# skmhrk1209/GANSynth

Measured on AMD Instinct MI355X. Metric: G+D step images/sec at 128x1024x2 mel+IF, higher is better.
Workload: dtype bf16; 1 GPU; BASELINE.json configs[1]: fully grown PGGAN 128x1024x2 G+D iteration (D update + G update, R1 + mode-seeking), per-GPU batch 8, random-init weights; global_batch=8, parallelism=dp1, launch=hipGraph replay, forked branches, forked_branches=True

## Files before the change

gansynth_amd/_lib.py:

```python
import ctypes
import os
from ctypes import c_char_p, c_double, c_float, c_int, c_int64, c_size_t, c_void_p, POINTER

_HERE = os.path.dirname(os.path.abspath(__file__))
LIB_PATH = os.path.join(_HERE, "libgansynth_hip.so")

GS_F32, GS_BF16 = 0, 1
ACT_NONE, ACT_LRELU, ACT_TANH = 0, 1, 2
ACT_LRELU_BITS, ACT_WRITE_BITS = 5, 16
PREP_CONV_FWD, PREP_CONV_BWD_DATA, PREP_CONVT_FWD, PREP_CONVT_BWD_DATA = 0, 1, 2, 3
CONV_FWD, CONV_BWD_DATA, CONV_BWD_WEIGHT = 0, 1, 2

P, I, F, L, Z = c_void_p, c_int, c_float, c_int64, c_size_t

SIGNATURES = {
    "gs_last_error": (c_char_p, []),
    "gs_version": (I, []),
    "gs_init": (I, []),
    "gs_streams_create": (I, [I, POINTER(P)]),
    "gs_streams_destroy": (I, [I, POINTER(P)]),
    "gs_prof_enable": (I, [I]),
    "gs_prof_collect": (I, [POINTER(c_int), POINTER(c_double), POINTER(c_double)]),
    "gs_prof_roofline": (I, [ctypes.c_double, ctypes.c_double, P, P, P]),
    "gs_prof_records": (I, [I, P, P, P, P, P]),
    "gs_comm_available": (I, []),
    "gs_comm_unique_id": (I, [P]),
    "gs_comm_init": (I, [POINTER(P), I, I, P]),
    "gs_comm_destroy": (I, [P]),
    "gs_comm_count": (I, [P, POINTER(I)]),
    "gs_allreduce_sum_f32": (I, [P, P, ctypes.c_int64, P]),
    "gs_comm_set_marker_us": (I, [P, ctypes.c_double]),
    "gs_broadcast_f32": (I, [P, P, ctypes.c_int64, I, P]),
    "gs_conv2d_workspace_bytes": (Z, [I, I, I, I, I, I, I, I, I]),
    "gs_conv2d_fwd": (I, [P, P, P, I, I, I, I, I, I, I, F, I, I, P, Z, P]),
    "gs_conv2d_fwd_bias_act": (I, [P, P, P, P, I, I, I, I, I, I, I, F, I, I, I, P, Z, P]),
    "gs_conv2d_bwd_data": (I, [P, P, P, I, I, I, I, I, I, I, F, I, I, P, Z, P]),
    "gs_conv2d_fwd_bias_act_norm": (I, [P, P, P, P, P, I, I, I, I, I, I, I, F, I, F, I, I, P, Z, P]),
    "gs_conv2d_transpose_s2_fwd_bias_act_norm": (I, [P, P, P, P, P, I, I, I, I, I, F, I, F, I, I, P, Z, P]),
    "gs_conv2d_fwd_mask": (I, [P, P, P, I, P, I, I, I, I, I, I, I, F, I, I, P, Z, P]),
    "gs_conv2d_bwd_data_mask": (I, [P, P, P, I, P, I, I, I, I, I, I, I, F, I, I, P, Z, P]),
    "gs_conv2d_bwd_weight": (I, [P, P, P, I, I, I, I, I, I, I, F, I, I, P, Z, P]),
    "gs_conv2d_bwd_weight_bias": (I, [P, P, P, P, I, I, I, I, I, I, I, F, I, I, P, Z, P]),
    "gs_conv2d_bwd_weight_bias_partial": (I, [P, P, P, P, I, I, I, I, I, I, I, F, I, I, P, Z, P, P]),
    "gs_conv2d_transpose_s2_bwd_weight_partial": (I, [P, P, P, I, I, I, I, I, F, I, I, P, Z, P, P]),
    "gs_wgrad_reduce_batch": (I, [P, I, P]),
    "gs_conv2d_bwd_weight_bias_multi": (I, [P, P, P, I, ctypes.c_uint, P, P, I, I, I, I, I, I, I, F, I, I, P, Z, P, P]),
    "gs_conv2d_transpose_s2_bwd_weight_multi": (I, [P, P, P, I, P, I, I, I, I, I, F, I, I, P, Z, P, P]),
    "gs_conv_wgrad_jobs_workspace_bytes": (Z, [P, I]),
    "gs_conv_wgrad_jobs": (I, [P, I, P, Z, P]),
    "gs_wgrad_cu_cap": (I, [I]),
    "gs_conv2d_transpose_s2_workspace_bytes": (Z, [I, I, I, I, I, I, I]),
    "gs_conv2d_transpose_s2_fwd": (I, [P, P, P, I, I, I, I, I, F, I, I, P, Z, P]),
    "gs_conv2d_transpose_s2_fwd_bias_act": (I, [P, P, P, P, I, I, I, I, I, F, I, I, I, P, Z, P]),
    "gs_conv2d_transpose_s2_bwd_data": (I, [P, P, P, I, I, I, I, I, F, I, I, P, Z, P]),
    "gs_conv2d_bwd_data_pnbwd_is_fused": (I, [I, I, I, I, I, I, I, I, I]),
    "gs_conv2d_fwd_pnbwdbwd_is_fused": (I, [I, I, I, I, I, I, I, I, I]),
    "gs_units_bias_act_to_nhwc": (I, [P, P, P, P, I, I, I, I, I, P]),
    "gs_nhwc_act_bwd_to_units": (I, [P, P, P, I, I, I, I, I, P]),
    "gs_conv2d_fwd_pnbwdbwd": (I, [P, P, P, P, I, F, P, P, I, I, I, I, I, I, I, F, I, I, P, Z, P]),
    "gs_conv2d_transpose_s2_fwd_pnbwdbwd": (I, [P, P, P, P, I, F, P, P, I, I, I, I, I, F, I, I, P, Z, P]),
    "gs_conv2d_bwd_data_pnbwd": (I, [P, P, P, P, I, F, P, I, I, I, I, I, I, I, F, I, I, P, Z, P]),
    "gs_conv2d_transpose_s2_bwd_data_pnbwd": (I, [P, P, P, P, I, F, P, I, I, I, I, I, F, I, I, P, Z, P]),
    "gs_conv2d_transpose_s2_bwd_weight": (I, [P, P, P, I, I, I, I, I, F, I, I, P, Z, P]),
    "gs_dense_fwd_workspace_bytes": (Z, [I, I, I]),
    "gs_dense_fwd": (I, [P, P, P, I, I, I, F, I, P, Z, P]),
    "gs_dense_fwd_bias_act": (I, [P, P, P, P, I, I, I, F, I, I, P, Z, P]),
    "gs_dense_fwd_bias_act_nhwc": (I, [P, P, P, P, I, I, I, I, F, I, I, P, Z, P]),
    "gs_dense_bwd_data": (I, [P, P, P, I, I, I, F, I, P]),
    "gs_dense_bwd_weight": (I, [P, P, P, I, I, I, F, I, I, P]),
    "gs_dense_fwd_nhwc": (I, [P, P, P, I, I, I, I, F, I, P, Z, P]),
    "gs_dense_bwd_data_nhwc": (I, [P, P, P, I, I, I, I, F, I, P]),
    "gs_dense_bwd_weight_nhwc": (I, [P, P, P, I, I, I, I, F, I, I, P]),
    "gs_embedding_fwd": (I, [P, P, P, I, I, I, F, I, P]),
    "gs_embedding_onehot_fwd": (I, [P, P, P, P, I, I, I, F, I, P]),
    "gs_embedding_bwd": (I, [P, P, P, I, I, I, F, I, P]),
    "gs_bias_act_fwd": (I, [P, P, P, L, I, I, I, P]),
    "gs_act_bwd": (I, [P, P, P, L, I, I, P]),
    "gs_act_bwd_bias": (I, [P, P, P, P, L, I, I, I, I, P, Z, P]),
    "gs_tanh_bwd_bwd": (I, [P, P, P, P, L, I, P]),
    "gs_channel_sum_workspace_bytes": (Z, [L, I]),
    "gs_channel_sum": (I, [P, P, L, I, I, I, P, Z, P]),
    "gs_bias_partial_rows": (I, [I, L, I, I]),
    "gs_channel_fold_batch_workspace_bytes": (Z, [P, I]),
# ... 99 lines not shown
```

gansynth_amd/config.py:

```python
import os

KNOBS = {
    "GS_TORCH_COLLECTIVES": ("operational", "gradient all-reduce through torch.distributed's communicator instead of the library's own (gs_comm_*)"),
    "GS_NO_GRAPH_ALLREDUCE": ("operational", "no RCCL collective inside captured graphs: eager all-reduce behind each replay (bench.DP_LADDER's tamer modes)"),
    "GS_FORK_PROBE": ("operational", "auto | always | never: probe a forked hipGraph replay in a child process before the first forked capture "
                                     "(auto: only on HIP builds the workaround was not debugged on, fork_probe._forked_replay_ok)"),
    "GS_FORK_PROBED": ("operational", "(set by the probe for child processes: ok | died)"),
    "GS_FORK_PROBE_TIMEOUT_S": ("operational", "budget of that probe, seconds (600)"),
    "GS_LEVEL_STREAMS": ("operational", "throw-away streams alive while a graph is instantiated (128; capture.Capture._leveled_queues)"),
    "GS_COMM_MARKER_US": ("operational", "tests / profiles at world size 1: the one-rank all-reduce becomes a kernel that holds its stream this long "
                                         "(read once per communicator, comm.RcclComm; gs_comm_set_marker_us)"),
    "GS_CAPTURE_MODE": ("operational", "debugging: force torch.cuda.graph's capture_error_mode"),
    "GS_DEBUG_POISON_WS": ("operational", "debugging: kernel workspaces start as NaN bit patterns"),
    "GS_CHECK_FUSION": ("operational", "debugging: every fused cross-node form also runs its unfused definition and the two are compared"),
    "GS_FORK_EAGER": ("operational", "tests: the forked branches with eager launches on two streams"),
    "GS_NO_FORK_MARKS": ("operational", "debugging: branches start where they are opened, not at their marks"),
    "GS_NO_FORK": ("schedule", "no parallel branches in the runs' graphs (5.9 against 5.2 ms; also taken when GPU_MAX_HW_QUEUES != 4 or the probe fails)"),
    "GS_NO_MERGED_RUNS": ("schedule", "part A of the generator run NOT inside the discriminator run's graph (5.13 against 4.99 ms)"),
    "GS_NO_FUSED_ITERATION": ("schedule", "two graphs per iteration with eager optimizer steps between them (neutral on one GPU; data parallel both "
                                          "all-reduces are then the last node of a graph)"),
    "GS_OVERLAP_REDUCE": ("schedule", "data parallel: round 4's four-graph iteration, each all-reduce on a forked branch beside part A of the other run "
                                      "(hides both collectives; +0.7 ms at world size 1)"),
    "GS_NO_OVERLAP_REDUCE": ("schedule", "(overrides GS_OVERLAP_REDUCE)"),
    "GS_DEBUG_DP_BUCKET": ("operational", "print the range the first message of a two-step discriminator all-reduce covers"),
    "GS_DP_BUCKET_D": ("schedule", "data parallel: the discriminator's gradient all-reduced in two steps, ~98 % of it beside the end of its backward (300-us stand-ins: -0.09 ... -0.14 ms fully grown, +0.15 in a fade-in)"),
    "GS_EARLY_FLUSH_DIV": ("schedule", "a layer is 'large' from 1/DIV of the full resolution's pixels (16)"),
    "GS_EARLY_FLUSH_CUS": ("schedule", "CUs the early weight-gradient contraction is sized for (192; 160 / 224 / 256 within noise, round 6)"),
    "GS_D_TAIL_LEVELS": ("schedule", "levels of the discriminator's tail run over [real; fake] as one batch when the runs do not fork (3)"),
    "GS_NO_EARLY_FLUSH": ("ablation", "weight gradients of the full-chip levels contracted at the end of the run only"),
    "GS_NO_DEFERRED_REDUCE": ("ablation", "every weight gradient contracted where autograd produces it"),
    "GS_NO_DEFERRED_FOLDS": ("ablation", "bias-gradient partial rows folded by their producers"),
    "GS_NO_WGRAD_GROUPS": ("ablation", "no grouped weight-gradient launches"),
    "GS_NO_SPLIT_G_LOSS": ("ablation", "the generator's loss as one launch over both halves: the mode-seeking second-order pass waits for the discriminator's forward"),
    "GS_NO_SPLIT_FINAL_FLUSH": ("ablation", "the final weight-gradient contraction of a run on one stream (HBM-bound and MFMA-bound jobs one after the other)"),
    "GS_NO_FUSED_LOSSES": ("ablation", "per-sample loss algebra in torch instead of the one-launch loss heads"),
    "GS_NO_D_TAIL_BATCH": ("ablation", "real and fake pass through the discriminator's tail separately (no-fork schedule)"),
    "GS_NO_FUSED_NORM": ("ablation", "pixel norm as its own node behind every generator conv"),
    "GS_NO_NORM_EPILOGUE": ("ablation", "no pixel norm in conv epilogues"),
    "GS_NO_NORM_BWD_EPILOGUE": ("ablation", "no previous-block norm backward in data-gradient epilogues"),
    "GS_NO_NORM_BWD2_EPILOGUE": ("ablation", "no second-order norm kernel in the forward-on-cotangent conv"),
    "GS_NO_NORM_BWD_BIAS": ("ablation", "bias sums outside the norm's backward"),
    "GS_NO_MASK_BITS": ("ablation", "leaky-relu masks read as the bf16 activations themselves, not as the sign bits stored behind them"),
    "GS_NO_PREMASK": ("ablation", "activation derivative never folded into the consuming data-gradient kernel"),
    "GS_NO_PREMASK_GRAPH": ("ablation", "... not across autograd nodes"),
    "GS_NO_PREMASK_GRAPH2": ("ablation", "... not in second-order graphs"),
    "GS_NO_PARAMS_ONLY": ("ablation", "leaf activations receive gradients like tf.gradients would not ask for"),
    "GS_NO_DERIVED_SLICES": ("ablation", "the 257-channel conv's weight slices copied on every use"),
# ... 19 lines not shown
```

gansynth_amd/csrc/conv_igemm.hip:

```cpp
#include <type_traits>
#include "conv_shared.h"
#include "gs_prof.h"

#ifndef GS_WGRAD_THIN_PREFETCH
#define GS_WGRAD_THIN_PREFETCH 1
#endif

extern "C" int gs_pixel_norm_fwd(const void* x, void* y, int64_t p, int c, float eps, int dtype, void* stream);
extern "C" int gs_pack_act_bits(void* z, int64_t p, int c, int dtype, void* stream);
extern "C" int gs_pixel_norm_bwd_fused(const void* g, const void* x, const void* addend, void* gx, int64_t p, int c, float eps, int pre_act, int post_act, int dtype,
                                       void* stream);
extern "C" int gs_pixel_norm_bwd_bwd_fused(const void* gg, const void* g, const void* x, void* out, void* out_g, int64_t p, int c, float eps, int pre_act,
                                           int dtype, void* stream);

namespace gs {

typedef float f32x16 __attribute__((ext_vector_type(16)));
typedef float f32x4 __attribute__((ext_vector_type(4)));
typedef __bf16 bf16x8 __attribute__((ext_vector_type(8)));


template <typename T> struct Mma;
template <> struct Mma<float> {
    typedef f32x4 frag_t;
// ... 1419 lines not shown
    if (slice < ntiles) {
        tile_setup(slice);
#pragma unroll
        for (int q = 0; q < NPIECE; ++q) issue_piece(q, 0);
    }
    constexpr int PPG = (NPIECE + NG - 1) / NG;
    for (int tile = slice; tile < ntiles; tile += nslices) {
        const bool more = tile + nslices < ntiles;
        wait_vmcnt(0);
        block_barrier();
        do_bias = bias_next;
        if (more) tile_setup(tile + nslices);
        const unsigned char* const xpl = lds_raw + buf * BUF + it * XPL;
        const unsigned char* const gpl = lds_raw + buf * BUF + 2 * XPL + ot * GPL;
        load_group(0, 0, xpl, gpl);
        __builtin_amdgcn_sched_barrier(0);
        static_for<NG>([&](auto gc) __attribute__((always_inline)) { GS_WG_GROUP_STEP(decltype(gc)::value, more, xpl, gpl, buf ^ 1); });
        block_barrier();
        buf ^= 1;
    }
    const long pstride = 9L * IC * OC + (with_bias ? OC : 0);
    if (bias_wave) {
        const float tot = swap32_sum(accb);
        if (hi == 0) part[(long)slice * pstride + 9L * IC * OC + oc0 + ot * 32 + l31] = tot;
    }
#pragma unroll
    for (int t = 0; t < 9; ++t) {
        float* dst = part + (long)slice * pstride + ((long)t * IC + ic0 + it * 32) * OC + oc0 + ot * 32 + l31;
#pragma unroll
        for (int r = 0; r < 16; ++r) dst[(long)((r & 3) + 8 * (r >> 2) + 4 * hi) * OC] = acc[t][r];
    }
}

#ifndef GS_SK_ROW128
#define GS_SK_ROW128 1
#endif
#ifndef GS_SK_FRONT_S1
#define GS_SK_FRONT_S1 0
#endif
#ifndef GS_SK_FRONT_S2
#define GS_SK_FRONT_S2 1
#endif
template <int MODE, int TW, bool SPEC>
__global__ __launch_bounds__(SPEC ? 512 : 256) void conv_wgrad_bf16_2x2_sk_kernel(const SkGroup g, float* __restrict__ part) {
    constexpr bool S2 = MODE == MODE_S2;
    constexpr int NP = S2 ? 64 : 256;
    constexpr int TH = NP / TW;
    constexpr int PH = patch_dim<MODE>(TH), PW = patch_dim<MODE>(TW);
    constexpr int S = S2 ? 2 : 1;
    constexpr bool R128 = GS_SK_ROW128 != 0;
    constexpr int XRG = R128 ? (PH * PW + 7) / 8 : (PH * PW + 15) / 16;
    constexpr int GRG = R128 ? NP / 8 : NP / 16;
    constexpr int XK = (XRG + 3) / 4, GK = GRG / 4;
    constexpr int XPL = R128 ? 0 : XK * 4096, GPL = R128 ? 0 : NP * 64;
    constexpr int XT = R128 ? XK * 4096 : 2 * XK * 4096, GT = NP * 128;
    constexpr int BUF = XT + GT;
    constexpr int NPIECE = R128 ? XK + GK : 2 * XK + 2 * GK;
    constexpr int XROWB = R128 ? 128 : 64, GROWB = XROWB;
    extern __shared__ __attribute__((aligned(16))) unsigned char lds_raw[];
    const unsigned a_base = (unsigned)(uintptr_t)lds_raw;

    const int tid = threadIdx.x;
    const int lane = tid & 63, hi = lane >> 5, l31 = lane & 31;
    const int wv8 = __builtin_amdgcn_readfirstlane(tid >> 6);
    const bool loader = SPEC && wv8 >= 4, issuer = !SPEC || loader, computer = !SPEC || !loader;
    const int wv = wv8 & 3;
    const int it = wv >> 1, ot = wv & 1;
    const int t_row = (lane & 15) >> 2;
    const int t_col = (((lane >> 4) & 1) * 16 + (lane & 3) * 4) * 2;
    const long nb = gridDim.x, total = g.total_units;
    const int U0 = (int)((blockIdx.x * total) / nb), U1 = (int)(((blockIdx.x + 1) * total) / nb);
    if (U0 >= U1) return;

    constexpr int RPP = R128 ? 8 : 16;
    const int p_row = R128 ? lane >> 3 : lane >> 2;
    int x_ly[XK], x_lx[XK], x_voff[XK], x_sw[XK];
#pragma unroll
// ... 167 lines not shown
                if (more) {
#pragma unroll
                    for (int q = 0; q < NPIECE; ++q) issue_piece(q, buf ^ 1);
                }
            } else {
                load_group(0, 0, xpl, gpl);
                __builtin_amdgcn_sched_barrier(0);
                static_for<NG>([&](auto gc) __attribute__((always_inline)) { GS_WG_GROUP_STEP(decltype(gc)::value, false, xpl, gpl, buf ^ 1); });
            }
        } else {
            load_group(0, 0, xpl, gpl);
            __builtin_amdgcn_sched_barrier(0);
            static_for<NG>([&](auto gc) __attribute__((always_inline)) { GS_WG_GROUP_STEP(decltype(gc)::value, more, xpl, gpl, buf ^ 1); });
        }
        block_barrier();
        buf ^= 1;
        if (leave && computer) {
            float* const dst0 = part + (long)(blockIdx.x + run_c) * GS_SK_PSTRIDE;
            if (bias_wave_c) {
                const float tot = swap32_sum(accb);
                if (hi == 0) dst0[9 * 4096 + ot * 32 + l31] = tot;
            }
            accb = 0.f;
#pragma unroll
            for (int t = 0; t < 9; ++t) {
                float* dst = dst0 + (t * 64 + it * 32) * 64 + ot * 32 + l31;
#pragma unroll
                for (int r = 0; r < 16; ++r) {
                    dst[((r & 3) + 8 * (r >> 2) + 4 * hi) * 64] = acc[t][r];
                    acc[t][r] = 0.f;
                }
            }
        }
    }
}

__global__ __launch_bounds__(256) void wgrad_sk_reduce_kernel(const SkGroup g, const float* __restrict__ part) {
    constexpr int L = 4, EPB = 64;
    __shared__ float4 red[256];
    const int r = blockIdx.y;
    int j = 0;
    while (j + 1 < g.njobs && r >= g.job[j + 1].run_base) ++j;
    const SkJob& q = g.job[j];
    const int ct = r - q.run_base;
    const int ic0 = (ct % q.n_ict) * 64, oc0 = (ct / q.n_ict) * 64;
    const long s0 = (long)q.unit_base + (long)ct * q.ntiles;
    const int b0 = sk_block_of(s0, g.nblocks, g.total_units), b1 = sk_block_of(s0 + q.ntiles - 1, g.nblocks, g.total_units);
    const int e = blockIdx.x * EPB + (threadIdx.x % EPB);
    const int sl = threadIdx.x / EPB;
    const bool live = e < GS_SK_PSTRIDE / 4;
    const bool is_bias = e >= 9 * 1024;
    if (blockIdx.x * EPB >= 9 * 1024 && !(q.gb && ic0 == 0)) return;
    const float* const base = part + (long)r * GS_SK_PSTRIDE + (long)e * 4;
    float4 a0 = make_float4(0.f, 0.f, 0.f, 0.f), a1 = a0, a2 = a0, a3 = a0;
    if (live) {
        int b = b0 + sl;
        for (; b + 3 * L <= b1; b += 4 * L) {
            const float4 v0 = *reinterpret_cast<const float4*>(base + (long)b * GS_SK_PSTRIDE);
            const float4 v1 = *reinterpret_cast<const float4*>(base + (long)(b + L) * GS_SK_PSTRIDE);
            const float4 v2 = *reinterpret_cast<const float4*>(base + (long)(b + 2 * L) * GS_SK_PSTRIDE);
            const float4 v3 = *reinterpret_cast<const float4*>(base + (long)(b + 3 * L) * GS_SK_PSTRIDE);
            a0.x += v0.x; a0.y += v0.y; a0.z += v0.z; a0.w += v0.w;
            a1.x += v1.x; a1.y += v1.y; a1.z += v1.z; a1.w += v1.w;
            a2.x += v2.x; a2.y += v2.y; a2.z += v2.z; a2.w += v2.w;
            a3.x += v3.x; a3.y += v3.y; a3.z += v3.z; a3.w += v3.w;
        }
        for (; b <= b1; b += L) {
            const float4 v0 = *reinterpret_cast<const float4*>(base + (long)b * GS_SK_PSTRIDE);
            a0.x += v0.x; a0.y += v0.y; a0.z += v0.z; a0.w += v0.w;
        }
    }
    a0.x += a2.x; a0.y += a2.y; a0.z += a2.z; a0.w += a2.w;
    a1.x += a3.x; a1.y += a3.y; a1.z += a3.z; a1.w += a3.w;
    red[threadIdx.x] = make_float4(a0.x + a1.x, a0.y + a1.y, a0.z + a1.z, a0.w + a1.w);
    __syncthreads();
    if (sl != 0 || !live) return;
    float4 s = make_float4(0.f, 0.f, 0.f, 0.f);
#pragma unroll
    for (int k = 0; k < L; ++k) {
        const float4 v = red[threadIdx.x + k * EPB];
        s.x += v.x; s.y += v.y; s.z += v.z; s.w += v.w;
    }
    if (is_bias) {
        if (!(q.gb && ic0 == 0)) return;
        float4* o = reinterpret_cast<float4*>(q.gb + oc0 + (e - 9 * 1024) * 4);
        const float4 old = q.accumulate ? *o : make_float4(0.f, 0.f, 0.f, 0.f);
        *o = make_float4(old.x + s.x, old.y + s.y, old.z + s.z, old.w + s.w);
        return;
    }
    const int t = e >> 10, i = (e >> 4) & 63, j4 = (e & 15) * 4;
    const float al = q.alpha;
    if (!q.transpose) {
        float4* o = reinterpret_cast<float4*>(q.gw + ((long)t * q.ICld + ic0 + i) * q.OC + oc0 + j4);
        const float4 old = q.accumulate ? *o : make_float4(0.f, 0.f, 0.f, 0.f);
        *o = make_float4(old.x + s.x * al, old.y + s.y * al, old.z + s.z * al, old.w + s.w * al);
    } else {
        const float v[4] = {s.x, s.y, s.z, s.w};
#pragma unroll
        for (int c = 0; c < 4; ++c) {
            float* o = q.gw + ((long)t * q.OC + oc0 + j4 + c) * q.IC + ic0 + i;
            *o = q.accumulate ? *o + v[c] * al : v[c] * al;
        }
    }
}


static int g_num_cus = 0;
static int num_cus() {
    if (g_num_cus == 0) {
        int dev = 0, n = 0;
        if (hipGetDevice(&dev) == hipSuccess && hipDeviceGetAttribute(&n, hipDeviceAttributeMultiprocessorCount, dev) == hipSuccess && n > 0)
            g_num_cus = n;
        else
            g_num_cus = 256;
    }
    return g_num_cus;
}
static int g_wgrad_cu_cap = 0;
static int wgrad_cus() {
    const int n = num_cus();
    return g_wgrad_cu_cap > 0 && g_wgrad_cu_cap < n ? g_wgrad_cu_cap : n;
}

#ifndef GS_MAX_BLOCKS_PER_CU
#define GS_MAX_BLOCKS_PER_CU 2
#endif
#ifndef GS_SMALL_D
#define GS_SMALL_D 2
#endif
template <typename T, int MODE, int A, int B, int TW, int TG, bool RESIDENT = false, int D = 2, int NORM = 0, int RB = 64, bool SPEC = false, bool BITS = false>
static int launch_igemm(ConvP p, hipStream_t st) {
    if constexpr (!BITS && sizeof(T) == 2 && NORM == 0) {
        if (p.mask_bits || p.bits_out) return launch_igemm<T, MODE, A, B, TW, TG, RESIDENT, D, NORM, RB, SPEC, true>(p, st);
    }
    constexpr int NP = 128 * B;
    constexpr int TH = NP / TW;
// ... 445 lines not shown
int wgrad_sk_tile_width(int Wb) {
    static const bool tw16 = getenv("GS_SK_TW16") != nullptr;
    return (Wb >= 32 || !tw16) ? 32 : 16;
}
void wgrad_sk_job_geometry(int mode, int tw, int N, SkJob& q) {
    const int np = mode == MODE_S2 ? 64 : 256;
    const int th = np / tw;
    q.tiles_x = cdiv(q.Wb, tw);
    q.tiles_y = cdiv(q.Hb, th);
    q.ntiles = N * q.tiles_x * q.tiles_y;
    q.n_ict = q.IC / 64;
    q.nct = q.n_ict * (q.OC / 64);
}
void wgrad_sk_plan(int mode, SkGroup& g) {
    long units = 0;
    int runs = 0;
    for (int j = 0; j < g.njobs; ++j) {
        g.job[j].unit_base = (int)units;
        g.job[j].run_base = runs;
        units += (long)g.job[j].nct * g.job[j].ntiles;
        runs += g.job[j].nct;
    }
    g.total_units = (int)units;
    g.total_runs = runs;
    static const int upb_env = getenv("GS_SK_UNITS_PER_BLOCK") ? atoi(getenv("GS_SK_UNITS_PER_BLOCK")) : 0;
    static const int upb2_env = getenv("GS_SK_UNITS_PER_BLOCK_S2") ? atoi(getenv("GS_SK_UNITS_PER_BLOCK_S2")) : 0;
    const int upb = mode == MODE_S2 ? (upb2_env > 0 ? upb2_env : 4) : (upb_env > 0 ? upb_env : 2);
    long nb = units / upb;
    if (nb > wgrad_cus()) nb = wgrad_cus();
    if (nb < 1) nb = 1;
    g.nblocks = (int)nb;
}
size_t wgrad_sk_bytes(const SkGroup& g) { return align256((size_t)(g.nblocks + g.total_runs) * GS_SK_PSTRIDE * sizeof(float)); }

int run_wgrad_sk(int mode, int tw, const SkGroup& g, void* ws, size_t ws_bytes, hipStream_t st) {
    if (g.njobs < 1 || g.njobs > GS_SK_MAX_JOBS) return fail(GS_ERR_ARG, "conv wgrad group: %d jobs", g.njobs);
    if (ws_bytes < wgrad_sk_bytes(g)) return fail(GS_ERR_WORKSPACE, "conv wgrad group: workspace %zu < %zu", ws_bytes, wgrad_sk_bytes(g));
    if ((long)g.total_units <= 0) return 0;
    float* part = reinterpret_cast<float*>(ws);
    double flops = 0.0, bytes = 0.0;
    int images = 0;
    for (int j = 0; j < g.njobs; ++j) {
        const SkJob& q = g.job[j];
        const int N = q.srcs.n_end[GS_WGRAD_MAX_SRC - 1];
        images += N;
        flops += 2.0 * 9.0 * (double)N * q.Hb * q.Wb * q.IC * q.OC;
        bytes += ((double)N * q.Hi * q.Wi * q.IC + (double)N * q.Hb * q.Wb * q.OC) * 2.0 + 9.0 * q.IC * q.OC * 4.0;
    }
    {
        ProfScope ps(st, flops, bytes, 20 + mode, g.njobs, tw, g.nblocks, g.total_units, g.total_runs, images, 1);
#define GS_WGSK(M, TWV, SP)                                                                                              \
    do {                                                                                                                \
        constexpr int np_ = (M == MODE_S2 ? 64 : 256), th_ = np_ / TWV;                                                 \
        constexpr int lds_ = 2 * (2 * ((((patch_dim<M>(th_) * patch_dim<M>(TWV) + 15) / 16 + 3) / 4) * 4096 + np_ * 64));  \
        auto kern_ = conv_wgrad_bf16_2x2_sk_kernel<M, TWV, SP>;                                                         \
        static bool set_ = false;                                                                                       \
        if (!set_) {                                                                                                    \
            if (hipFuncSetAttribute(reinterpret_cast<const void*>(kern_), hipFuncAttributeMaxDynamicSharedMemorySize, lds_) != hipSuccess) \
                return fail(GS_ERR_HIP, "conv wgrad group: cannot reserve %d bytes of dynamic LDS", lds_);              \
            set_ = true;                                                                                                \
        }                                                                                                               \
        hipLaunchKernelGGL(kern_, dim3((unsigned)g.nblocks), dim3(SP ? 512 : 256), lds_, st, g, part);                  \
    } while (0)
        static const int spec_env = getenv("GS_SK_SPEC") ? atoi(getenv("GS_SK_SPEC")) : 0;
        const bool spec = spec_env == 1 || (spec_env == 2 && mode == MODE_S1);
        if (spec) {
            if (mode == MODE_S1) { if (tw == 32) GS_WGSK(MODE_S1, 32, true); else GS_WGSK(MODE_S1, 16, true); }
            else { if (tw == 32) GS_WGSK(MODE_S2, 32, true); else GS_WGSK(MODE_S2, 16, true); }
        } else {
            if (mode == MODE_S1) { if (tw == 32) GS_WGSK(MODE_S1, 32, false); else GS_WGSK(MODE_S1, 16, false); }
            else { if (tw == 32) GS_WGSK(MODE_S2, 32, false); else GS_WGSK(MODE_S2, 16, false); }
        }
#undef GS_WGSK
    }
    GS_CHECK_LAUNCH();
    hipLaunchKernelGGL(wgrad_sk_reduce_kernel, dim3((GS_SK_PSTRIDE / 4 + 63) / 64, (unsigned)g.total_runs), dim3(256), 0, st, g, part);
    GS_CHECK_LAUNCH();
    return 0;
}

}

extern "C" int gs_wgrad_cu_cap(int cap) {
    const int was = gs::g_wgrad_cu_cap;
    gs::g_wgrad_cu_cap = cap < 0 ? 0 : cap;
    return was;
}
extern "C" int gs_prof_enable(int on) {
    gs::g_prof.on = on != 0;
    gs::g_prof.burst = on > 1 ? on : 1;
    gs::g_prof.used = 0;
    gs::g_prof.flops = 0.0;
    return 0;
}

extern "C" int gs_prof_roofline(double peak_tflops, double peak_gbps, double* total_bytes, double* roof_ms, double* roof_ms_hbm_bound) {
    double bytes = 0.0, roof = 0.0, roof_hbm = 0.0;
    for (int i = 0; i < gs::g_prof.used; ++i) {
        if (gs::g_prof.ldesc[i][0] >= 10) continue;
        const double tf = gs::g_prof.lflops[i] / (peak_tflops * 1e12) * 1e3, tb = gs::g_prof.lbytes[i] / (peak_gbps * 1e9) * 1e3;
        bytes += gs::g_prof.lbytes[i];
        roof += tf > tb ? tf : tb;
        if (tb >= tf) roof_hbm += tb;
    }
    if (total_bytes) *total_bytes = bytes;
    if (roof_ms) *roof_ms = roof;
    if (roof_ms_hbm_bound) *roof_ms_hbm_bound = roof_hbm;
    return 0;
}

extern "C" int gs_prof_records(int max_records, int* n, double* ms, double* flops, double* bytes, int* desc) {
    int k = 0;
    for (int i = 0; i < gs::g_prof.used && k < max_records; ++i, ++k) {
// ... 29 lines not shown
```

gansynth_amd/kernels.py:

```python
import contextlib
import ctypes
import os

import numpy as np
import torch

from . import config
from . import _lib
from ._lib import GS_BF16, GS_F32

CL = torch.channels_last


def _dt(t):
    if t.dtype == torch.float32:
        return GS_F32
    if t.dtype == torch.bfloat16:
        return GS_BF16
    raise TypeError(f"unsupported activation dtype {t.dtype}")


def _act(x):
    if x.dim() == 4:
        return x if x.is_contiguous(memory_format=CL) else x.contiguous(memory_format=CL)
# ... 30 lines not shown
            and t.untyped_storage().nbytes() == t.numel() * 2 + t.numel() // 8)


def _mask_act(mask, mask_act):
    return _lib.ACT_LRELU_BITS if (mask_act == _lib.ACT_LRELU and _has_bits(mask)) else int(mask_act)


def _stream():
    return ctypes.c_void_p(torch.cuda.current_stream().cuda_stream)


_POISON = config.flag("GS_DEBUG_POISON_WS")


def _ws(nbytes, device):
    if _POISON:
        return torch.full((max(int(nbytes), 256),), 0xFF, dtype=torch.uint8, device=device)
    return torch.empty(max(int(nbytes), 256), dtype=torch.uint8, device=device)


def _rows_cols(x):
    if x.dim() == 4:
        n, c, h, w = x.shape
        return n * h * w, c
    return x.shape[0], x.shape[1]


class HipKernels(object):
    def __init__(self):
        self.lib = _lib.load()
        if not torch.cuda.is_available():
            raise _lib.GansynthHipError("gansynth_amd needs a HIP device (torch.cuda.is_available() is False)")
        _lib.check(self.lib.gs_init(), "gs_init")
        self._param_ranges = []
        self._wcache = {}
        self._prep_tables = {}
        self._derived = {}
        self._folds = None
        self._pending = None
        self._guarding = False
        self._last_writer = {}
        self._early = None
        self._seen = None
        self._expected = {}
        self._tag = None
        self._complete = None

    def register_param_buffer(self, flat):
        self._param_ranges.append([flat.data_ptr(), flat.numel() * flat.element_size(), 0])

    def invalidate_weights(self, flat=None):
        ptr = None if flat is None else flat.data_ptr()
        for rng in self._param_ranges:
            if ptr is None or rng[0] <= ptr < rng[0] + rng[1]:
                rng[2] += 1

    def _weight_ws(self, w, tag, nbytes, plan=None):
        ptr = w.data_ptr()
        rng = next((r for r in self._param_ranges if r[0] <= ptr < r[0] + r[1]), None)
        if rng is None:
            return _ws(nbytes, w.device), 0
        key, stamp = (ptr, tag), (rng[2], w._version)
        ent = self._wcache.get(key)
        if ent is not None and ent[0].numel() >= nbytes:
            if ent[1] == stamp:
                return ent[0], 1
# ... 1095 lines not shown
```

include/gansynth_hip.h:

```cpp
#ifndef GANSYNTH_HIP_H
#define GANSYNTH_HIP_H

#include <stddef.h>
#include <stdint.h>

#ifdef __cplusplus
extern "C" {
#endif

enum { GS_F32 = 0, GS_BF16 = 1 };
enum { GS_OK = 0, GS_ERR_ARG = -1, GS_ERR_HIP = -2, GS_ERR_UNSUPPORTED = -3, GS_ERR_WORKSPACE = -4 };
enum { GS_ACT_NONE = 0, GS_ACT_LRELU = 1, GS_ACT_TANH = 2 };
enum { GS_ACT_LRELU_BITS = 5, GS_ACT_WRITE_BITS = 16 };
enum { GS_CONV_FWD = 0, GS_CONV_BWD_DATA = 1, GS_CONV_BWD_WEIGHT = 2 };

const char* gs_last_error(void);
int gs_version(void);
int gs_init(void);
int gs_streams_create(int n, void** streams);
int gs_streams_destroy(int n, void** streams);

int gs_prof_enable(int on);
int gs_prof_collect(int* launches, double* total_ms, double* total_flops);
int gs_prof_roofline(double peak_tflops, double peak_gbps, double* total_bytes, double* roof_ms, double* roof_ms_hbm_bound);
// ... 65 lines not shown
    int32_t ic_ld;
} GsWgradReduce;
int gs_conv2d_bwd_weight_bias_partial(const void* x, const void* gy, float* gw_hwio, float* gb, int n, int h, int w, int ci, int co,
                                      int ksize, int stride, float alpha, int accumulate, int dtype, void* ws, size_t ws_bytes,
                                      GsWgradReduce* pending, void* stream);
int gs_conv2d_transpose_s2_bwd_weight_partial(const void* x, const void* gy, float* gw_hwio, int n, int h, int w, int ci, int co,
                                              float alpha, int accumulate, int dtype, void* ws, size_t ws_bytes,
                                              GsWgradReduce* pending, void* stream);
int gs_wgrad_reduce_batch(const GsWgradReduce* pending, int n, void* stream);
#define GS_WGRAD_MAX_SOURCES 4
int gs_conv2d_bwd_weight_bias_multi(const void* const* xs, const void* const* gys, const int* ns, int nsrc, unsigned bias_mask, float* gw_hwio,
                                    float* gb, int n, int h, int w, int ci, int co, int ksize, int stride, float alpha, int accumulate,
                                    int dtype, void* ws, size_t ws_bytes, GsWgradReduce* pending, void* stream);
int gs_conv2d_transpose_s2_bwd_weight_multi(const void* const* xs, const void* const* gys, const int* ns, int nsrc, float* gw_hwio, int n, int h,
                                            int w, int ci, int co, float alpha, int accumulate, int dtype, void* ws, size_t ws_bytes,
                                            GsWgradReduce* pending, void* stream);

typedef struct GsWgradJob {
    const void* x[GS_WGRAD_MAX_SOURCES];
    const void* gy[GS_WGRAD_MAX_SOURCES];
    int32_t n[GS_WGRAD_MAX_SOURCES];
    int32_t nsrc;
    uint32_t bias_mask;
    float* gw;
    float* gb;
    int32_t h, w, ci, co, ksize, stride, transposed;
    float alpha;
    int32_t accumulate, dtype;
    int32_t gw_ci_stride;
} GsWgradJob;
size_t gs_conv_wgrad_jobs_workspace_bytes(const GsWgradJob* jobs, int njobs);
int gs_conv_wgrad_jobs(const GsWgradJob* jobs, int njobs, void* ws, size_t ws_bytes, void* stream);
int gs_wgrad_cu_cap(int cap);

enum { GS_PREP_CONV_FWD = 0, GS_PREP_CONV_BWD_DATA = 1, GS_PREP_CONVT_FWD = 2, GS_PREP_CONVT_BWD_DATA = 3 };
typedef struct GsPrepDesc {
    const float* w_hwio;
    void* ws;
    int32_t map, ci, co, ksize, stride, dtype;
} GsPrepDesc;
int gs_weight_prep_batch(const GsPrepDesc* descs, int n, void* stream);

size_t gs_dense_fwd_workspace_bytes(int b, int in, int out);
int gs_dense_fwd(const void* x, const float* w, void* y, int b, int in, int out, float alpha, int dtype,
                 void* ws, size_t ws_bytes, void* stream);
int gs_dense_bwd_data(const void* gy, const float* w, void* gx, int b, int in, int out, float alpha, int dtype, void* stream);
int gs_dense_bwd_weight(const void* x, const void* gy, float* gw, int b, int in, int out, float alpha, int accumulate, int dtype,
                        void* stream);
int gs_dense_fwd_bias_act(const void* x, const float* w, const float* bias, void* y, int b, int in, int out, float alpha, int act,
                          int dtype, void* ws, size_t ws_bytes, void* stream);
int gs_dense_fwd_nhwc(const void* x, const float* w, void* y, int b, int c, int hw, int out, float alpha, int dtype,
                      void* ws, size_t ws_bytes, void* stream);
int gs_dense_fwd_bias_act_nhwc(const void* x, const float* w, const float* bias, void* y, int b, int c, int hw, int out, float alpha,
                               int act, int dtype, void* ws, size_t ws_bytes, void* stream);
int gs_dense_bwd_data_nhwc(const void* gy, const float* w, void* gx, int b, int c, int hw, int out, float alpha, int dtype, void* stream);
int gs_dense_bwd_weight_nhwc(const void* x, const void* gy, float* gw, int b, int c, int hw, int out, float alpha, int accumulate,
                             int dtype, void* stream);

int gs_embedding_fwd(const int64_t* idx, const float* w, void* y, int b, int rows, int units, float alpha, int dtype, void* stream);
int gs_embedding_onehot_fwd(const void* labels, const float* w, void* y, int64_t* idx_out, int b, int rows, int units, float alpha, int dtype, void* stream);
int gs_embedding_bwd(const int64_t* idx, const void* gy, float* gw, int b, int rows, int units, float alpha, int dtype, void* stream);

int gs_bias_act_fwd(const void* x, const float* bias, void* y, int64_t p, int c, int act, int dtype, void* stream);
int gs_act_bwd(const void* g, const void* y, void* gx, int64_t numel, int act, int dtype, void* stream);
int gs_units_bias_act_to_nhwc(const void* y, const float* bias, const void* mask, void* z, int n, int c, int hw, int act, int dtype, void* stream);
int gs_nhwc_act_bwd_to_units(const void* g, const void* z, void* gu, int n, int c, int hw, int act, int dtype, void* stream);
// ... 90 lines not shown
```

Measured before the change: 1622 images/sec.

## Fold stream-K weight-gradient partials inside the launch via last-block tickets

Stream-K grouped weight-gradient kernels now take atomic per-run tickets, and the last block to finish a run of up to 8 partials sums and stores that run itself. The separate reduce launch then covers only the runs too long to fold, or is skipped entirely. This removes a kernel launch and the extra pass over partials for most runs. In exchange it adds a memset of the ticket counters, atomics with fences, and a serial fold done by one block per run, which can lengthen the kernel's tail.

```diff
diff --git a/gansynth_amd/_lib.py b/gansynth_amd/_lib.py
--- a/gansynth_amd/_lib.py
+++ b/gansynth_amd/_lib.py
@@ -49,6 +49,7 @@
     "gs_conv_wgrad_jobs_workspace_bytes": (Z, [P, I]),
     "gs_conv_wgrad_jobs": (I, [P, I, P, Z, P]),
     "gs_wgrad_cu_cap": (I, [I]),
+    "gs_wgrad_sk_fold": (I, [I]),
     "gs_conv2d_transpose_s2_workspace_bytes": (Z, [I, I, I, I, I, I, I]),
     "gs_conv2d_transpose_s2_fwd": (I, [P, P, P, I, I, I, I, I, F, I, I, P, Z, P]),
     "gs_conv2d_transpose_s2_fwd_bias_act": (I, [P, P, P, P, I, I, I, I, I, F, I, I, I, P, Z, P]),
diff --git a/gansynth_amd/config.py b/gansynth_amd/config.py
--- a/gansynth_amd/config.py
+++ b/gansynth_amd/config.py
@@ -13,6 +13,8 @@
     "GS_CAPTURE_MODE": ("operational", "debugging: force torch.cuda.graph's capture_error_mode"),
     "GS_DEBUG_POISON_WS": ("operational", "debugging: kernel workspaces start as NaN bit patterns"),
     "GS_CHECK_FUSION": ("operational", "debugging: every fused cross-node form also runs its unfused definition and the two are compared"),
+    "GS_SK_INLAUNCH_FOLD": ("operational", "grouped weight gradients: runs of at most this many partials are folded inside the launch by their last "
+                                           "block (default 8, DESIGN.md 6.7); 0: always the separate fold launch; same bits either way (gs_wgrad_sk_fold)"),
     "GS_FORK_EAGER": ("operational", "tests: the forked branches with eager launches on two streams"),
     "GS_NO_FORK_MARKS": ("operational", "debugging: branches start where they are opened, not at their marks"),
     "GS_NO_FORK": ("schedule", "no parallel branches in the runs' graphs (5.9 against 5.2 ms; also taken when GPU_MAX_HW_QUEUES != 4 or the probe fails)"),
diff --git a/gansynth_amd/csrc/conv_igemm.hip b/gansynth_amd/csrc/conv_igemm.hip
--- a/gansynth_amd/csrc/conv_igemm.hip
+++ b/gansynth_amd/csrc/conv_igemm.hip
@@ -1475,6 +1475,119 @@
     }
 }
 
+struct SkRun {
+    int j, ic0, oc0, b0, b1;
+};
+__device__ __forceinline__ SkRun sk_run_of(const SkGroup& g, int r) {
+    SkRun rn;
+    int j = 0;
+    while (j + 1 < g.njobs && r >= g.job[j + 1].run_base) ++j;
+    const SkJob& q = g.job[j];
+    const int ct = r - q.run_base;
+    rn.j = j;
+    rn.ic0 = (ct % q.n_ict) * 64;
+    rn.oc0 = (ct / q.n_ict) * 64;
+    const long s0 = (long)q.unit_base + (long)ct * q.ntiles;
+    rn.b0 = sk_block_of(s0, g.nblocks, g.total_units);
+    rn.b1 = sk_block_of(s0 + q.ntiles - 1, g.nblocks, g.total_units);
+    return rn;
+}
+__device__ __forceinline__ void sk_add4(float4& a, const float4& v) { a.x += v.x; a.y += v.y; a.z += v.z; a.w += v.w; }
+__device__ __forceinline__ float4 sk_lane_sum(const float* base, int b, int b1) {
+    constexpr int L = 4;
+    float4 a0 = make_float4(0.f, 0.f, 0.f, 0.f), a1 = a0, a2 = a0, a3 = a0;
+    for (; b + 3 * L <= b1; b += 4 * L) {
+        const float4 v0 = *reinterpret_cast<const float4*>(base + (long)b * GS_SK_PSTRIDE);
+        const float4 v1 = *reinterpret_cast<const float4*>(base + (long)(b + L) * GS_SK_PSTRIDE);
+        const float4 v2 = *reinterpret_cast<const float4*>(base + (long)(b + 2 * L) * GS_SK_PSTRIDE);
+        const float4 v3 = *reinterpret_cast<const float4*>(base + (long)(b + 3 * L) * GS_SK_PSTRIDE);
+        sk_add4(a0, v0); sk_add4(a1, v1); sk_add4(a2, v2); sk_add4(a3, v3);
+    }
+    for (; b <= b1; b += L) sk_add4(a0, *reinterpret_cast<const float4*>(base + (long)b * GS_SK_PSTRIDE));
+    sk_add4(a0, a2);
+    sk_add4(a1, a3);
+    return make_float4(a0.x + a1.x, a0.y + a1.y, a0.z + a1.z, a0.w + a1.w);
+}
+__device__ __forceinline__ void sk_store_quad(const SkJob& q, int e, int ic0, int oc0, const float4 s) {
+    if (e >= 9 * 1024) {
+        if (!(q.gb && ic0 == 0)) return;
+        float4* o = reinterpret_cast<float4*>(q.gb + oc0 + (e - 9 * 1024) * 4);
+        const float4 old = q.accumulate ? *o : make_float4(0.f, 0.f, 0.f, 0.f);
+        *o = make_float4(old.x + s.x, old.y + s.y, old.z + s.z, old.w + s.w);
+        return;
+    }
+    const int t = e >> 10, i = (e >> 4) & 63, j4 = (e & 15) * 4;
+    const float al = q.alpha;
+    if (!q.transpose) {
+        float4* o = reinterpret_cast<float4*>(q.gw + ((long)t * q.ICld + ic0 + i) * q.OC + oc0 + j4);
+        const float4 old = q.accumulate ? *o : make_float4(0.f, 0.f, 0.f, 0.f);
+        *o = make_float4(old.x + s.x * al, old.y + s.y * al, old.z + s.z * al, old.w + s.w * al);
+    } else {
+        const float v[4] = {s.x, s.y, s.z, s.w};
+#pragma unroll
+        for (int c = 0; c < 4; ++c) {
+            float* o = q.gw + ((long)t * q.OC + oc0 + j4 + c) * q.IC + ic0 + i;
+            *o = q.accumulate ? *o + v[c] * al : v[c] * al;
+        }
+    }
+}
+#define GS_SK_FOLD_FLAT 8
+template <int NT, int QUADS, int NP>
+__device__ __forceinline__ void sk_fold_flat(const SkJob& q, const float* slot0, int nq, const SkRun& rn, int tid) {
+    const float4 z = make_float4(0.f, 0.f, 0.f, 0.f);
+    for (int e0 = tid; e0 < nq; e0 += NT * QUADS) {
+        float4 v[QUADS][NP];
+#pragma unroll
+        for (int i = 0; i < QUADS; ++i) {
+            const int e = min(e0 + i * NT, nq - 1);
+#pragma unroll
+            for (int k = 0; k < NP; ++k) v[i][k] = *reinterpret_cast<const float4*>(slot0 + (long)k * GS_SK_PSTRIDE + (long)e * 4);
+        }
+#pragma unroll
+        for (int i = 0; i < QUADS; ++i) {
+            const int e = e0 + i * NT;
+            if (e >= nq) continue;
+            float4 s = z;
+#pragma unroll
+            for (int sl = 0; sl < 4; ++sl) {
+                float4 a0 = z, a1 = z;
+                if (sl < NP) sk_add4(a0, v[i][sl < NP ? sl : 0]);
+                if (sl + 4 < NP) sk_add4(a0, v[i][sl + 4 < NP ? sl + 4 : 0]);
+                sk_add4(a0, z);
+                sk_add4(a1, z);
+                sk_add4(s, make_float4(a0.x + a1.x, a0.y + a1.y, a0.z + a1.z, a0.w + a1.w));
+            }
+            sk_store_quad(q, e, rn.ic0, rn.oc0, s);
+        }
+    }
+}
+template <int NT, int QUADS>
+__device__ __forceinline__ void sk_fold_run(const SkGroup& g, const float* part, int r, const SkRun& rn, int tid) {
+    const SkJob& q = g.job[rn.j];
+    const int nq = (q.gb && rn.ic0 == 0) ? GS_SK_PSTRIDE / 4 : 9 * 1024;
+    const float* const slot0 = part + (long)(r + rn.b0) * GS_SK_PSTRIDE;
+    switch (rn.b1 - rn.b0 + 1) {
+        case 1: sk_fold_flat<NT, QUADS, 1>(q, slot0, nq, rn, tid); return;
+        case 2: sk_fold_flat<NT, QUADS, 2>(q, slot0, nq, rn, tid); return;
+        case 3: sk_fold_flat<NT, QUADS, 3>(q, slot0, nq, rn, tid); return;
+        case 4: sk_fold_flat<NT, QUADS, 4>(q, slot0, nq, rn, tid); return;
+        case 5: sk_fold_flat<NT, QUADS, 5>(q, slot0, nq, rn, tid); return;
+        case 6: sk_fold_flat<NT, QUADS, 6>(q, slot0, nq, rn, tid); return;
+        case 7: sk_fold_flat<NT, QUADS, 7>(q, slot0, nq, rn, tid); return;
+        case 8: sk_fold_flat<NT, QUADS, 8>(q, slot0, nq, rn, tid); return;
+        default: break;
+    }
+    static_assert(GS_SK_FOLD_FLAT == 8, "one case per flat partial count");
+    const float4 z = make_float4(0.f, 0.f, 0.f, 0.f);
+    for (int e = tid; e < nq; e += NT) {
+        const float* const base = part + (long)r * GS_SK_PSTRIDE + (long)e * 4;
+        float4 s = z;
+#pragma unroll
+        for (int sl = 0; sl < 4; ++sl) sk_add4(s, sk_lane_sum(base, rn.b0 + sl, rn.b1));
+        sk_store_quad(q, e, rn.ic0, rn.oc0, s);
+    }
+}
+
 #ifndef GS_SK_ROW128
 #define GS_SK_ROW128 1
 #endif
@@ -1485,7 +1598,7 @@
 #define GS_SK_FRONT_S2 1
 #endif
 template <int MODE, int TW, bool SPEC>
-__global__ __launch_bounds__(SPEC ? 512 : 256) void conv_wgrad_bf16_2x2_sk_kernel(const SkGroup g, float* __restrict__ part) {
+__global__ __launch_bounds__(SPEC ? 512 : 256) void conv_wgrad_bf16_2x2_sk_kernel(const SkGroup g, float* part, unsigned* run_tickets, int fold_m) {
     constexpr bool S2 = MODE == MODE_S2;
     constexpr int NP = S2 ? 64 : 256;
     constexpr int TH = NP / TW;
@@ -1719,47 +1832,49 @@
                 }
             }
         }
-    }
-}
-
-__global__ __launch_bounds__(256) void wgrad_sk_reduce_kernel(const SkGroup g, const float* __restrict__ part) {
+        if (leave && fold_m > 0) {
+            const SkRun rn = sk_run_of(g, run_c);
+            const int np = rn.b1 - rn.b0 + 1;
+            if (np <= fold_m) {
+                volatile int* const flag = reinterpret_cast<volatile int*>(lds_raw + (buf ^ 1) * BUF);
+                if (computer) wait_vmcnt(0);
+                block_barrier();
+                if (tid == 0) {
+                    __builtin_amdgcn_fence(__ATOMIC_RELEASE, "agent");
+                    asm volatile("s_waitcnt vmcnt(0)" ::: "memory");
+                    const unsigned ticket = __hip_atomic_fetch_add(run_tickets + run_c, 1u, __ATOMIC_RELAXED, __HIP_MEMORY_SCOPE_AGENT);
+                    const int last = ticket == (unsigned)(np - 1);
+                    if (last) {
+                        __builtin_amdgcn_fence(__ATOMIC_ACQUIRE, "agent");
+                        asm volatile("s_waitcnt vmcnt(0)" ::: "memory");
+                        __hip_atomic_store(run_tickets + run_c, 0u, __ATOMIC_RELAXED, __HIP_MEMORY_SCOPE_AGENT);
+                    }
+                    *flag = last;
+                }
+                block_barrier();
+                const int last = __builtin_amdgcn_readfirstlane(*flag);
+                if (last && tid < 256) sk_fold_run<256, SPEC ? 1 : 4>(g, part, run_c, rn, tid);
+            }
+        }
+    }
+}
+
+__global__ __launch_bounds__(256) void wgrad_sk_reduce_kernel(const SkGroup g, const float* __restrict__ part, int fold_m, int run_lo) {
     constexpr int L = 4, EPB = 64;
     __shared__ float4 red[256];
-    const int r = blockIdx.y;
-    int j = 0;
-    while (j + 1 < g.njobs && r >= g.job[j + 1].run_base) ++j;
-    const SkJob& q = g.job[j];
-    const int ct = r - q.run_base;
-    const int ic0 = (ct % q.n_ict) * 64, oc0 = (ct / q.n_ict) * 64;
-    const long s0 = (long)q.unit_base + (long)ct * q.ntiles;
-    const int b0 = sk_block_of(s0, g.nblocks, g.total_units), b1 = sk_block_of(s0 + q.ntiles - 1, g.nblocks, g.total_units);
+    const int r = run_lo + blockIdx.y;
+    const SkRun rn = sk_run_of(g, r);
+    if (fold_m > 0 && rn.b1 - rn.b0 + 1 <= fold_m) return;
+    const SkJob& q = g.job[rn.j];
+    const int ic0 = rn.ic0;
     const int e = blockIdx.x * EPB + (threadIdx.x % EPB);
     const int sl = threadIdx.x / EPB;
     const bool live = e < GS_SK_PSTRIDE / 4;
-    const bool is_bias = e >= 9 * 1024;
     if (blockIdx.x * EPB >= 9 * 1024 && !(q.gb && ic0 == 0)) return;
     const float* const base = part + (long)r * GS_SK_PSTRIDE + (long)e * 4;
-    float4 a0 = make_float4(0.f, 0.f, 0.f, 0.f), a1 = a0, a2 = a0, a3 = a0;
-    if (live) {
-        int b = b0 + sl;
-        for (; b + 3 * L <= b1; b += 4 * L) {
-            const float4 v0 = *reinterpret_cast<const float4*>(base + (long)b * GS_SK_PSTRIDE);
-            const float4 v1 = *reinterpret_cast<const float4*>(base + (long)(b + L) * GS_SK_PSTRIDE);
-            const float4 v2 = *reinterpret_cast<const float4*>(base + (long)(b + 2 * L) * GS_SK_PSTRIDE);
-            const float4 v3 = *reinterpret_cast<const float4*>(base + (long)(b + 3 * L) * GS_SK_PSTRIDE);
-            a0.x += v0.x; a0.y += v0.y; a0.z += v0.z; a0.w += v0.w;
-            a1.x += v1.x; a1.y += v1.y; a1.z += v1.z; a1.w += v1.w;
-            a2.x += v2.x; a2.y += v2.y; a2.z += v2.z; a2.w += v2.w;
-            a3.x += v3.x; a3.y += v3.y; a3.z += v3.z; a3.w += v3.w;
-        }
-        for (; b <= b1; b += L) {
-            const float4 v0 = *reinterpret_cast<const float4*>(base + (long)b * GS_SK_PSTRIDE);
-            a0.x += v0.x; a0.y += v0.y; a0.z += v0.z; a0.w += v0.w;
-        }
-    }
-    a0.x += a2.x; a0.y += a2.y; a0.z += a2.z; a0.w += a2.w;
-    a1.x += a3.x; a1.y += a3.y; a1.z += a3.z; a1.w += a3.w;
-    red[threadIdx.x] = make_float4(a0.x + a1.x, a0.y + a1.y, a0.z + a1.z, a0.w + a1.w);
+    float4 lane = make_float4(0.f, 0.f, 0.f, 0.f);
+    if (live) lane = sk_lane_sum(base, rn.b0 + sl, rn.b1);
+    red[threadIdx.x] = lane;
     __syncthreads();
     if (sl != 0 || !live) return;
     float4 s = make_float4(0.f, 0.f, 0.f, 0.f);
@@ -1768,27 +1883,7 @@
         const float4 v = red[threadIdx.x + k * EPB];
         s.x += v.x; s.y += v.y; s.z += v.z; s.w += v.w;
     }
-    if (is_bias) {
-        if (!(q.gb && ic0 == 0)) return;
-        float4* o = reinterpret_cast<float4*>(q.gb + oc0 + (e - 9 * 1024) * 4);
-        const float4 old = q.accumulate ? *o : make_float4(0.f, 0.f, 0.f, 0.f);
-        *o = make_float4(old.x + s.x, old.y + s.y, old.z + s.z, old.w + s.w);
-        return;
-    }
-    const int t = e >> 10, i = (e >> 4) & 63, j4 = (e & 15) * 4;
-    const float al = q.alpha;
-    if (!q.transpose) {
-        float4* o = reinterpret_cast<float4*>(q.gw + ((long)t * q.ICld + ic0 + i) * q.OC + oc0 + j4);
-        const float4 old = q.accumulate ? *o : make_float4(0.f, 0.f, 0.f, 0.f);
-        *o = make_float4(old.x + s.x * al, old.y + s.y * al, old.z + s.z * al, old.w + s.w * al);
-    } else {
-        const float v[4] = {s.x, s.y, s.z, s.w};
-#pragma unroll
-        for (int c = 0; c < 4; ++c) {
-            float* o = q.gw + ((long)t * q.OC + oc0 + j4 + c) * q.IC + ic0 + i;
-            *o = q.accumulate ? *o + v[c] * al : v[c] * al;
-        }
-    }
+    sk_store_quad(q, e, rn.ic0, rn.oc0, s);
 }
 
 
@@ -2300,12 +2395,33 @@
     g.nblocks = (int)nb;
 }
 size_t wgrad_sk_bytes(const SkGroup& g) { return align256((size_t)(g.nblocks + g.total_runs) * GS_SK_PSTRIDE * sizeof(float)); }
+#ifndef GS_SK_FOLD_DEFAULT
+#define GS_SK_FOLD_DEFAULT 8
+#endif
+static int g_sk_fold = GS_SK_FOLD_DEFAULT;
 
 int run_wgrad_sk(int mode, int tw, const SkGroup& g, void* ws, size_t ws_bytes, hipStream_t st) {
     if (g.njobs < 1 || g.njobs > GS_SK_MAX_JOBS) return fail(GS_ERR_ARG, "conv wgrad group: %d jobs", g.njobs);
     if (ws_bytes < wgrad_sk_bytes(g)) return fail(GS_ERR_WORKSPACE, "conv wgrad group: workspace %zu < %zu", ws_bytes, wgrad_sk_bytes(g));
     if ((long)g.total_units <= 0) return 0;
     float* part = reinterpret_cast<float*>(ws);
+    const int fold_m = g.total_runs <= GS_SK_PSTRIDE ? g_sk_fold : 0;
+    unsigned* const tickets = reinterpret_cast<unsigned*>(part + (size_t)(g.nblocks + g.total_runs - 1) * GS_SK_PSTRIDE);
+    int run_lo = g.total_runs, run_hi = -1;
+    for (int j = 0; j < g.njobs; ++j) {
+        const SkJob& q = g.job[j];
+        for (int ct = 0; ct < q.nct; ++ct) {
+            const long s0 = (long)q.unit_base + (long)ct * q.ntiles;
+            const int np = sk_block_of(s0 + q.ntiles - 1, g.nblocks, g.total_units) - sk_block_of(s0, g.nblocks, g.total_units) + 1;
+            if (fold_m > 0 && np <= fold_m) continue;
+            const int r = q.run_base + ct;
+            if (r < run_lo) run_lo = r;
+            if (r > run_hi) run_hi = r;
+        }
+    }
+    if (fold_m > 0 && run_hi - run_lo + 1 < g.total_runs) {
+        if (hipMemsetAsync(tickets, 0, (size_t)g.total_runs * sizeof(unsigned), st) != hipSuccess) return fail(GS_ERR_HIP, "conv wgrad group: cannot zero the run counters");
+    }
     double flops = 0.0, bytes = 0.0;
     int images = 0;
     for (int j = 0; j < g.njobs; ++j) {
@@ -2328,7 +2444,7 @@
                 return fail(GS_ERR_HIP, "conv wgrad group: cannot reserve %d bytes of dynamic LDS", lds_);              \
             set_ = true;                                                                                                \
         }                                                                                                               \
-        hipLaunchKernelGGL(kern_, dim3((unsigned)g.nblocks), dim3(SP ? 512 : 256), lds_, st, g, part);                  \
+        hipLaunchKernelGGL(kern_, dim3((unsigned)g.nblocks), dim3(SP ? 512 : 256), lds_, st, g, part, tickets, fold_m);  \
     } while (0)
         static const int spec_env = getenv("GS_SK_SPEC") ? atoi(getenv("GS_SK_SPEC")) : 0;
         const bool spec = spec_env == 1 || (spec_env == 2 && mode == MODE_S1);
@@ -2342,11 +2458,19 @@
 #undef GS_WGSK
     }
     GS_CHECK_LAUNCH();
-    hipLaunchKernelGGL(wgrad_sk_reduce_kernel, dim3((GS_SK_PSTRIDE / 4 + 63) / 64, (unsigned)g.total_runs), dim3(256), 0, st, g, part);
-    GS_CHECK_LAUNCH();
+    if (run_hi >= run_lo) {
+        hipLaunchKernelGGL(wgrad_sk_reduce_kernel, dim3((GS_SK_PSTRIDE / 4 + 63) / 64, (unsigned)(run_hi - run_lo + 1)), dim3(256), 0, st, g, part, fold_m, run_lo);
+        GS_CHECK_LAUNCH();
+    }
     return 0;
 }
 
+}
+
+extern "C" int gs_wgrad_sk_fold(int max_partials) {
+    const int was = gs::g_sk_fold;
+    gs::g_sk_fold = max_partials < 0 ? 0 : max_partials;
+    return was;
 }
 
 extern "C" int gs_wgrad_cu_cap(int cap) {
diff --git a/gansynth_amd/kernels.py b/gansynth_amd/kernels.py
--- a/gansynth_amd/kernels.py
+++ b/gansynth_amd/kernels.py
@@ -86,6 +86,8 @@
         if not torch.cuda.is_available():
             raise _lib.GansynthHipError("gansynth_amd needs a HIP device (torch.cuda.is_available() is False)")
         _lib.check(self.lib.gs_init(), "gs_init")
+        if config.value("GS_SK_INLAUNCH_FOLD") is not None:
+            self.lib.gs_wgrad_sk_fold(int(config.value("GS_SK_INLAUNCH_FOLD")))
         self._param_ranges = []
         self._wcache = {}
         self._prep_tables = {}
diff --git a/include/gansynth_hip.h b/include/gansynth_hip.h
--- a/include/gansynth_hip.h
+++ b/include/gansynth_hip.h
@@ -121,6 +121,7 @@
 size_t gs_conv_wgrad_jobs_workspace_bytes(const GsWgradJob* jobs, int njobs);
 int gs_conv_wgrad_jobs(const GsWgradJob* jobs, int njobs, void* ws, size_t ws_bytes, void* stream);
 int gs_wgrad_cu_cap(int cap);
+int gs_wgrad_sk_fold(int max_partials);
 
 enum { GS_PREP_CONV_FWD = 0, GS_PREP_CONV_BWD_DATA = 1, GS_PREP_CONVT_FWD = 2, GS_PREP_CONVT_BWD_DATA = 3 };
 typedef struct GsPrepDesc {
```

Result: slower. 1560 images/sec (-3.8%).
